# mattoverby/admm-elastic-sca

Hardware: AMD Instinct MI355X
Metric: ADMM iters/sec x #elements, 1M-tet Neo-Hookean; 1/2/4/8 MI355X (higher is better)
Workload: dtype f64

## Files before the change

admm-elastic-sca_amd/csrc/abi_setup.inc:

```

static void reset_frames(admm_hip_ctx *ctx) {
    for (int j = 0; j < ADMM_MAX_SHAPES; ++j) {
        for (int k = 0; k < 12; ++k) ctx->shapes.frame[j][k] = (k == 0 || k == 4 || k == 8) ? 1.0 : 0.0;
        ctx->shapes.framed[j] = 0;
    }
}

int admm_hip_create(admm_hip_ctx **out, int device_id) {
    if (!out) return ADMM_ERR_ARG;
    *out = nullptr;
    admm_hip_ctx *ctx = new admm_hip_ctx();
    ctx->device_id = device_id;
    if (device_id >= 0) {
        int count = 0;
        hipError_t e = hipGetDeviceCount(&count);
        if (e != hipSuccess || count <= device_id) {
            fprintf(stderr, "admm_hip: no HIP device %d (%s, %d devices) -- refusing to run without a GPU\n", device_id, hipGetErrorString(e), count);
            delete ctx;
            return ADMM_ERR_HIP;
        }
        if (hipSetDevice(device_id) != hipSuccess) { delete ctx; return ADMM_ERR_HIP; }
        if (hipStreamCreate(&ctx->stream) != hipSuccess) { delete ctx; return ADMM_ERR_HIP; }
        ctx->own_stream = true;
    }
// ... 6 lines not shown
    ctx->graph_enabled = false;
#endif
    if (const char *g = getenv("ADMM_HIP_GRAPH_COMM")) ctx->graph_comm = atoi(g) != 0;
    if (const char *g = getenv("ADMM_HIP_BWD_NW")) { const int v = atoi(g); if (v == 4 || v == 8 || v == 16) ctx->bwd_nw = v; }
    if (const char *g = getenv("ADMM_HIP_FWD_SMALL_K")) ctx->fwd_small_k = atoi(g);
    if (const char *g = getenv("ADMM_HIP_BWD_SMALL_K")) ctx->bwd_small_k = atoi(g);
    if (const char *g = getenv("ADMM_HIP_TREE_SEARCH")) ctx->tree_search = atoi(g) != 0;
    if (const char *g = getenv("ADMM_HIP_STATE_DIRECT")) ctx->state_direct_max_nodes = atoi(g);
    if (const char *g = getenv("ADMM_HIP_LOCAL_MULTI")) ctx->local_multi = atoi(g) != 0;
    if (const char *g = getenv("ADMM_HIP_TOP_BWD_ALL")) ctx->top_bwd_needed_only = atoi(g) == 0;
    if (const char *g = getenv("ADMM_HIP_ROOT_FUSE_K")) ctx->root_fuse_k = std::min(atoi(g), (int)admm_dev::ROOT_KCHUNK);
    if (const char *g = getenv("ADMM_HIP_FRAME_GRAPH")) ctx->frame_graph_on = atoi(g) != 0;
    if (const char *g = getenv("ADMM_HIP_BWD_SMALL_NW")) { const int v = atoi(g); if (v == 2 || v == 4 || v == 8 || v == 16) ctx->bwd_small_nw = v; }
    if (const char *g = getenv("ADMM_HIP_XCD")) ctx->xcd_min_supernodes = atoi(g);
    if (const char *g = getenv("ADMM_HIP_TET_ORDER")) ctx->tet_order = atoi(g) != 0;
    if (const char *g = getenv("ADMM_HIP_TET_ORDER_MIN")) ctx->tet_order_min_blocks = atoi(g);
    if (const char *g = getenv("ADMM_HIP_FUSE_ANCHORS")) ctx->fuse_anchor_tail = atoi(g) != 0;
    if (const char *g = getenv("ADMM_HIP_FACTOR")) ctx->device_factor = std::string(g) != "host";
    if (const char *g = getenv("ADMM_HIP_BWD_CW2_MIN")) ctx->bwd_cw2_min_cols = atoi(g);
    if (const char *g = getenv("ADMM_HIP_BWD_CW2_MAX")) ctx->bwd_cw2_max_cols = atoi(g);
    if (const char *g = getenv("ADMM_HIP_PRERED")) ctx->tet_prered = atoi(g) != 0;
    if (const char *g = getenv("ADMM_HIP_STATE_ZEROCOPY")) ctx->state_zero_copy = atoi(g) != 0;
    if (const char *g = getenv("ADMM_HIP_TPB")) { const int v = atoi(g); if (v == 4 || v == 8 || v == 16 || v == 32 || v == 64) ctx->tet_tpb = v; }
    if (const char *g = getenv("ADMM_HIP_KEEP_Z")) ctx->keep_z_user = atoi(g) != 0;
    if (const char *g = getenv("ADMM_HIP_BWD_NW_MIN_COLS")) ctx->bwd_nw_min_cols = atoi(g);
    if (const char *g = getenv("ADMM_HIP_FWD_NW16_TILES")) ctx->fwd_nw16_max_tiles = atoi(g);
    if (const char *g = getenv("ADMM_HIP_FWD_NW4")) ctx->fwd_nw4_kmax = atoi(g);
    if (const char *g = getenv("ADMM_HIP_FWD_NW8")) ctx->fwd_nw8_kmax = atoi(g);
    if (const char *g = getenv("ADMM_HIP_DENSE_MAX")) ctx->dense_max = atoi(g);
    if (const char *g = getenv("ADMM_HIP_ROOT_INVERSE")) ctx->root_inverse = atoi(g) != 0;
    if (const char *g = getenv("ADMM_HIP_DIST_TOP")) ctx->dist_top_wanted = atoi(g) != 0 ? 1 : 0;
    if (const char *g = getenv("ADMM_HIP_DIST_TOP_MIN_NODES")) ctx->dist_top_min_nodes = atoi(g);
    if (const char *g = getenv("ADMM_HIP_SWEEP_FUSE")) ctx->sweep_fuse = atoi(g) != 0;
    *out = ctx;
    return ADMM_OK;
}

void admm_hip_destroy(admm_hip_ctx *ctx) {
    if (!ctx) return;
    if (ctx->device_id >= 0) {
        (void)hipSetDevice(ctx->device_id);
        (void)hipDeviceSynchronize();
        free_device(ctx);
        for (hipEvent_t e : ctx->evpool) (void)hipEventDestroy(e);
        for (hipEvent_t e : ctx->evpool_prev) (void)hipEventDestroy(e);
        comm_release(ctx);
        for (double *h : {ctx->h_gen_dx, ctx->h_gen_u, ctx->h_gen_z, ctx->h_gen_q}) if (h) (void)hipHostFree(h);
        if (ctx->gen_ev) (void)hipEventDestroy(ctx->gen_ev);
        if (ctx->h_state) (void)hipHostFree(ctx->h_state);
        if (ctx->state_in_ev) (void)hipEventDestroy(ctx->state_in_ev);
        if (ctx->own_stream && ctx->stream) (void)hipStreamDestroy(ctx->stream);
    }
    delete ctx;
}

const char *admm_hip_last_error(const admm_hip_ctx *ctx) { return ctx ? ctx->err.c_str() : "null context"; }

int admm_hip_set_stream(admm_hip_ctx *ctx, void *s) {
    if (!ctx || ctx->device_id < 0) return ADMM_ERR_ARG;
    if (ctx->stream) { HIPCHK(hipSetDevice(ctx->device_id)); (void)hipStreamSynchronize(ctx->stream); }
    if (ctx->own_stream && ctx->stream) (void)hipStreamDestroy(ctx->stream);
    ctx->own_stream = false;
    ctx->stream = (hipStream_t)s;
    if (!s) { HIPCHK(hipStreamCreate(&ctx->stream)); ctx->own_stream = true; }
    return ADMM_OK;
}
// ... 664 lines not shown
```

admm-elastic-sca_amd/csrc/ctx.hpp:

```cpp
#pragma once
#include <hip/hip_runtime_api.h>

#include <algorithm>
#include <chrono>
#include <cmath>
#include <cstdarg>
#include <cstdio>
#include <cstring>
#include <numeric>
#include <string>
#include <vector>

#include "../../include/admm_hip.h"
#include "factor.hpp"
#include "dev_types.hpp"
#include "mesh_host.hpp"

namespace admm_lib {

inline double now_s() { return std::chrono::duration<double>(std::chrono::steady_clock::now().time_since_epoch()).count(); }

struct Batch {
    int kind = 0, n_total = 0, n_local = 0;
    std::vector<int32_t> local;
// ... 125 lines not shown
    int root_sn = -1, root_k = 0, root_first = 0, root_r0 = 0, root_r1 = 0; int64_t root_foff = 0;
    bool tet_order = true; int tet_order_min_blocks = 3072;
    int64_t frames = 0;
    int merge_small = 0;
    bool fuse_anchor_tail = true;
    bool device_factor = true, device_numeric = false;
    bool keep_z = true, keep_z_user = true;
    bool state_zero_copy = true;
    int tet_tpb = 0;
    bool tet_prered = true;
    int n_comm_top = 0, n_comm_slots = 0;
    int *d_comm_top = nullptr, *d_comm_slots = nullptr; unsigned char *d_comm_mine = nullptr, *d_base_mask = nullptr, *d_keep_mask = nullptr;
    double *d_comm_buf = nullptr;
    bool root_inverse = true;
    int dense_max = 2048; bool dense = false; std::vector<double> Ainv; double *d_ainv = nullptr;
    bool graph_enabled = true, graph_forced = false; hipGraph_t iter_graph = nullptr; hipGraphExec_t iter_exec = nullptr;
    bool frame_graph_on = true; hipGraph_t frame_graph = nullptr; hipGraphExec_t frame_exec = nullptr; int frame_iters = 0, last_step_iters = -1;
    bool local_multi = true;
    int state_direct_max_nodes = 12288; double *h_state = nullptr, *h_state_dev = nullptr; size_t h_state_cap = 0; int *d_iperm = nullptr; hipEvent_t state_in_ev = nullptr; bool state_in_pending = false;
    std::vector<std::pair<const char *, size_t> > pinned;
    std::vector<double> bounce;
    bool tree_search = true;
    bool top_bwd_needed_only = true;
    int root_fuse_k = 2048;
    int fwd_small_k = 64, bwd_small_k = 64;
    int bwd_cw2_min_cols = 8192, bwd_cw2_max_cols = 16384;
    int bwd_nw = 8, bwd_small_nw = 4;
    int xcd_min_supernodes = 16;
    int bwd_nw_min_cols = 4096, fwd_nw16_max_tiles = 512;
    int fwd_nw4_kmax = 200, fwd_nw8_kmax = 400;
    bool sweep_fuse = true;
    int fuse_cut = -1, n_fuse = 0, fuse_lds = 0;
    int *d_fuse_rec = nullptr; int64_t *d_fuse_off = nullptr;
    int64_t graph_launches = 0;
    bool graphs_stale = false;
    bool graph_comm = false;
    bool res_on = false, res_ready = false;
    double tol_r = 0.0, tol_s = 0.0; int check_every = 1;
    double *d_res = nullptr; int res_cap = 0, res_n = 0;
    double *d_res_slots = nullptr, *d_res_s = nullptr, *d_res_partial = nullptr; int res_partial_n = 0;
    bool en_ready = false; double *d_en_out = nullptr, *d_en_npart = nullptr; long long *d_en_cnt = nullptr;
    bool obj_on = false; int obj_cap = 0, obj_n = 0; double *d_obj = nullptr;
    bool gr_ready = false, gr_csr_ready = false; double *d_gr_cf = nullptr, *d_gr_out = nullptr;
    int *d_gr_ptr[2] = {nullptr, nullptr}, *d_gr_stride[2] = {nullptr, nullptr}; long long *d_gr_off[2] = {nullptr, nullptr};
    bool rx_ready = false; double *d_rx_el = nullptr, *d_rx_node = nullptr, *d_rx_part = nullptr; int *d_rx_blk = nullptr; long long *d_rx_count = nullptr; void *d_rx_rec = nullptr;
    int *d_rx_ptr[2] = {nullptr, nullptr}, *d_rx_stride[2] = {nullptr, nullptr}; long long *d_rx_off[2] = {nullptr, nullptr};
    int aa_m = 0, aa_cap_m = 0, aa_nblk = 0, aa_log_cap = 0, aa_log_n = 0; long long aa_T = 0; bool aa_ran = false;
    void *d_aa_seg = nullptr, *d_aa_state = nullptr; admm_hip_acceleration_record *d_aa_log = nullptr;
    double *d_aa_sin = nullptr, *d_aa_ring = nullptr, *d_aa_part = nullptr;

    admm_hip_project_fn project_hook = nullptr; void *project_user = nullptr;
    int64_t n_gen_rows = 0;
    double *d_gen_dx = nullptr, *d_gen_q = nullptr;
    double *h_gen_dx = nullptr, *h_gen_u = nullptr, *h_gen_z = nullptr, *h_gen_q = nullptr;
    std::vector<double> h_gen_u_prev, h_gen_z_prev; double *d_gen_q2 = nullptr, *d_gen_r2 = nullptr;
    hipEvent_t gen_ev = nullptr;
    bool timing = false; int timing_stride = 1; int ev_timed = 0; int timing_frame = 0;
    std::vector<hipEvent_t> evpool;
    size_t ev_used = 0; int ev_iters = 0; bool ev_pending = false;
    std::vector<hipEvent_t> evpool_prev; size_t ev_used_prev = 0; int ev_iters_prev = 0, ev_timed_prev = 0; bool ev_pending_prev = false;
    admm_hip_timing last_timing{};
};

namespace admm_lib {

int fail(admm_hip_ctx *c, int code, const char *fmt, ...);
// ... 40 lines not shown
```

admm-elastic-sca_amd/csrc/kernels_global.hpp:

```cpp
#pragma once
#include <hip/hip_runtime.h>
#include <stdint.h>
#include "dev_types.hpp"

namespace admm_dev {


__global__ void prologue_kernel(int ndof, double dt, Gravity gr, const double *__restrict__ x, double *__restrict__ v,
                                const double *__restrict__ m, double *__restrict__ mxbar, double *__restrict__ xcur) {
    const int i = blockIdx.x * blockDim.x + threadIdx.x;
    if (i >= ndof) return;
    const int c = i % 3;
    double vi = v[i];
    for (int k = 0; k < gr.n; ++k) vi += (dt * gr.g[k][c]);
    v[i] = vi;
    const double xb = x[i] + dt * vi;
    mxbar[i] = m[i] * xb;
    xcur[i] = xb;
}

__global__ void xbar_kernel(int ndof, double dt, const double *__restrict__ x, const double *__restrict__ v,
                            const double *__restrict__ m, double *__restrict__ mxbar, double *__restrict__ xcur) {
    const int i = blockIdx.x * blockDim.x + threadIdx.x;
    if (i >= ndof) return;
    const double xb = x[i] + dt * v[i];
    mxbar[i] = m[i] * xb;
    xcur[i] = xb;
}

__global__ void explicit_const_kernel(int n, const int *__restrict__ idx, double dt, double gx, double gy, double gz, double *__restrict__ v) {
    const int i = blockIdx.x * blockDim.x + threadIdx.x;
    if (i >= n) return;
    const int node = idx ? idx[i] : i;
    v[3 * (size_t)node] += (dt * gx); v[3 * (size_t)node + 1] += (dt * gy); v[3 * (size_t)node + 2] += (dt * gz);
}

// ... 587 lines not shown
                    for (int c = 0; c < CW; ++c) { acc[c][0] += pf[c] * v[0]; acc[c][1] += pf[c] * v[1]; acc[c][2] += pf[c] * v[2]; }
                    q += 64;
                }
                for (; q < rc; q += 64) {
                    const int i = r0 + q;
                    double p[CW];
#pragma unroll
                    for (int c = 0; c < CW; ++c) p[c] = (j0 + c < k && i >= j0 + c) ? Pj[i + (size_t)f * c] : 0.0;
                    const double *v = &vs[3 * q];
#pragma unroll
                    for (int c = 0; c < CW; ++c) { acc[c][0] += p[c] * v[0]; acc[c][1] += p[c] * v[1]; acc[c][2] += p[c] * v[2]; }
                }
                for (; q < rc; q += 64) {
                    const int i = r0 + q;
                    const double *v = &vs[3 * q];
#pragma unroll
                    for (int c = 0; c < CW; ++c) { const double p = (j0 + c < k && i >= j0 + c) ? Pj[i + (size_t)f * c] : 0.0; acc[c][0] += p * v[0]; acc[c][1] += p * v[1]; acc[c][2] += p * v[2]; }
                }
            }
        }
    }
    double v[3 * CW];
#pragma unroll
    for (int c = 0; c < CW; ++c) { v[3 * c] = acc[c][0]; v[3 * c + 1] = acc[c][1]; v[3 * c + 2] = acc[c][2]; }
    int base = 0, cnt = 3 * CW;
    wave_sum_transpose<3 * CW, 32>(v, lane, base, cnt);
    if (cnt >= 1) {
        const int c = base / 3, m = base - 3 * c;
        if (j0 + c < k) X[3 * (size_t)(first + j0 + c) + m] = v[0];
    }
    ADMM_SWEEP_STAMP(2);
}

template <bool CG2>
__global__ __launch_bounds__(256) void root_gather_kernel(int k, int first, int64_t foff, FactorDev F, const double *__restrict__ y, const double *__restrict__ C, double *__restrict__ T, double *__restrict__ Xzero = nullptr) {
    const int j = blockIdx.x * 256 + threadIdx.x;
    if (j >= k) return;
    if (Xzero) { Xzero[3 * (size_t)j] = 0.0; Xzero[3 * (size_t)j + 1] = 0.0; Xzero[3 * (size_t)j + 2] = 0.0; }
    double s0, s1, s2;
    child_sum<CG2>(F, foff + j, C, s0, s1, s2);
    const double *src = y + 3 * (size_t)(first + j);
    double *t = T + 3 * (size_t)j;
    t[0] = src[0] - s0; t[1] = src[1] - s1; t[2] = src[2] - s2;
}

__global__ __launch_bounds__(256) void dense_solve_kernel(int n, const double *__restrict__ Ainv, const double *__restrict__ b, double *__restrict__ X) {
    const int wave = threadIdx.x >> 6, lane = threadIdx.x & 63;
    const int i = blockIdx.x * 4 + wave;
    if (i >= n) return;
    const double *row = Ainv + (size_t)i * n;
    double v[3] = {0.0, 0.0, 0.0};
    int j = lane;
    for (; j + 448 < n; j += 512) {
        double a[8];
#pragma unroll
        for (int q = 0; q < 8; ++q) a[q] = row[j + 64 * q];
#pragma unroll
        for (int q = 0; q < 8; ++q) { const double *bj = b + 3 * (size_t)(j + 64 * q); v[0] += a[q] * bj[0]; v[1] += a[q] * bj[1]; v[2] += a[q] * bj[2]; }
    }
    for (; j + 192 < n; j += 256) {
        double a[4];
#pragma unroll
        for (int q = 0; q < 4; ++q) a[q] = row[j + 64 * q];
#pragma unroll
        for (int q = 0; q < 4; ++q) { const double *bj = b + 3 * (size_t)(j + 64 * q); v[0] += a[q] * bj[0]; v[1] += a[q] * bj[1]; v[2] += a[q] * bj[2]; }
    }
// ... 61 lines not shown
```

admm-elastic-sca_amd/csrc/launch.inc:

```

int max_lbfgs_iters(const Batch &b) { return b.max_iter; }

#ifdef ADMM_TET_PROFILE
float *g_trace_base; int g_trace_cap, g_trace_n, g_trace_count;
void tet_trace_next(hipStream_t st) {
    float *p = (g_trace_base && g_trace_count < g_trace_cap) ? g_trace_base + 2 * (size_t)g_trace_count * g_trace_n : nullptr;
    ++g_trace_count;
    hipMemcpyToSymbolAsync(HIP_SYMBOL(admm_dev::g_tet_trace), &p, sizeof(p), 0, hipMemcpyHostToDevice, st);
}
#endif
bool friction_on(const admm_hip_ctx *ctx) {
    for (int q = 0; q < ctx->shapes.n; ++q) if (ctx->shapes.mu[q] > 0.0) return true;
    return false;
}

bool moving_friction_on(const admm_hip_ctx *ctx) {
    for (int q = 0; q < ctx->shapes.n; ++q) {
        const int id = ctx->shapes.type[q] == ADMM_SHAPE_MESH ? (int)ctx->shapes.par[q][3] : -1;
        const admm_hip_ctx::MeshMove *mv = id >= 0 && id < (int)ctx->mesh_move.size() ? &ctx->mesh_move[id] : nullptr;
        if (mv && !ctx->mesh_role[id].body_nodes.empty() && mv->body_mu > 0.0) return true;
        if (!(ctx->shapes.mu[q] > 0.0)) continue;
        if (mv && mv->has_vel) return true;
        for (int k = 0; k < 9; ++k) if (ctx->shapes.motion[q][k] != 0.0) return true;
    }
// ... 340 lines not shown
                    return NWB != 2 || CW == 4;
                }); });
            }
        };
        if (ctx->n_fuse)
            hipLaunchKernelGGL(solve_fwd_subtree_kernel, dim3(ctx->n_fuse), dim3(64 * SUB_WAVES), ctx->fuse_lds, ctx->stream, (const int *)ctx->d_fuse_rec,
                               (const int64_t *)ctx->d_fuse_off, (const double *)ctx->d_panels, (const double *)ctx->d_y, ctx->d_w, ctx->d_c);
        forward(ctx->levels, ctx->stream);
        if (!ctx->levels_top.empty()) {
            const int n = ctx->n_comm_top + ctx->n_comm_slots;
            if (ex0) HIPCHK(hipEventRecord(ex0, ctx->stream));
            if (n > 0) {
                hipLaunchKernelGGL(shard_pack_kernel, dim3((n + 255) / 256), dim3(256), 0, ctx->stream, ctx->n_comm_top, (const int *)ctx->d_comm_top, ctx->n_comm_slots,
                                   (const int *)ctx->d_comm_slots, (const unsigned char *)ctx->d_comm_mine, (const double *)ctx->d_y, (const double *)ctx->d_c, ctx->d_comm_buf);
                TRY(do_allreduce(ctx, ctx->d_comm_buf, 3 * (int64_t)n));
                hipLaunchKernelGGL(shard_unpack_kernel, dim3((n + 255) / 256), dim3(256), 0, ctx->stream, ctx->n_comm_top, (const int *)ctx->d_comm_top, ctx->n_comm_slots,
                                   (const int *)ctx->d_comm_slots, (const double *)ctx->d_comm_buf, ctx->d_y, ctx->d_c);
            }
            if (ex1) HIPCHK(hipEventRecord(ex1, ctx->stream));
            if (ctx->dist_top) {
                const int k = ctx->root_k, nr = ctx->root_r1 - ctx->root_r0;
                double *T = ctx->d_w + 3 * (size_t)ctx->root_first, *Xr = ctx->d_xcur + 3 * (size_t)ctx->root_first;
                hipLaunchKernelGGL((root_gather_kernel<CG2>), dim3((k + 255) / 256), dim3(256), 0, ctx->stream, k, ctx->root_first, ctx->root_foff, F, (const double *)ctx->d_y, (const double *)ctx->d_c, T, Xr);
                if (nr > 0) hipLaunchKernelGGL((root_product_kernel<false, false>), dim3((nr + ROOT_ROWS - 1) / ROOT_ROWS), dim3(64 * ROOT_ROWS), 0, ctx->stream, k, nr, root_inv_ld(k),
                                               (const double *)(ctx->d_panels + ctx->dev_root_inv_off[ctx->root_sn]), (const double *)T, Xr + 3 * (size_t)ctx->root_r0, 0, (int64_t)0, F, (const double *)nullptr);
                if (ex2) HIPCHK(hipEventRecord(ex2, ctx->stream));
                TRY(do_allreduce(ctx, Xr, 3 * (int64_t)k));
                if (ex3) HIPCHK(hipEventRecord(ex3, ctx->stream));
            } else forward(ctx->levels_top, ctx->stream);
        }
        if (mid) HIPCHK(hipEventRecord(mid, ctx->stream));
        if (!ctx->levels_top.empty() && !ctx->dist_top) backward(ctx->levels_top, ctx->stream);
        backward(ctx->levels, ctx->stream);
        HIPCHK(hipGetLastError());
        if (bad_pair) return fail(ctx, ADMM_ERR_STATE, "backward sweep: no kernel for a level's (columns per wave, waves per block) pair");
        return ADMM_OK;
    };
    return F.cg4 ? sweeps(std::true_type{}) : sweeps(std::false_type{});
}

int shard_sync_x(admm_hip_ctx *ctx) {
    if (ctx->levels_top.empty()) return ADMM_OK;
    const int n3 = 3 * ctx->n_nodes;
    hipLaunchKernelGGL(admm_dev::shard_mask_nodes_kernel, dim3((n3 + 255) / 256), dim3(256), 0, ctx->stream, ctx->n_nodes, (const unsigned char *)ctx->d_keep_mask, ctx->d_xcur);
    TRY(do_allreduce(ctx, ctx->d_xcur, (int64_t)n3));
    HIPCHK(hipGetLastError());
    return ADMM_OK;
}


int ensure_residual_buffers(admm_hip_ctx *ctx, int iters) {
    if (ctx->res_ready && iters <= ctx->res_cap) return ADMM_OK;
    HIPCHK(hipSetDevice(ctx->device_id));
    if (!ctx->res_ready) {
        int64_t slots = 0; int maxn = 0;
        for (Batch &b : ctx->batches) {
            if (b.kind == ADMM_KIND_GENERIC) {
                std::vector<double> coef(b.g_sval.size());
                for (size_t i = 0; i < coef.size(); ++i) { const double w = b.g_roww[b.g_srow_b[i]]; coef[i] = b.g_sval[i] * (w * w); }
                TRY(upload(ctx, &b.d_g_scoef_res, coef));
                slots += b.g_lslots;
                continue;
            }
            const int rows = ADMM_KIND_ROWS[b.kind], nl = std::max(b.n_local, 1);
            b.res_fused = ((b.kind >= ADMM_KIND_TET_LINEAR && b.kind <= ADMM_KIND_TET_STVK) || b.kind == ADMM_KIND_ANCHOR) && (b.prered || getenv("ADMM_HIP_RES_UNFUSED") == nullptr);
            if (b.res_fused) {
// ... 113 lines not shown
```

admm-elastic-sca_amd/csrc/upload.inc:

```

template <class T> std::vector<T> permute_nodes(const std::vector<T> &h, const std::vector<int> &perm, int comps) {
    std::vector<T> o(h.size());
    for (size_t i = 0; i < perm.size(); ++i) for (int c = 0; c < comps; ++c) o[comps * i + c] = h[comps * (size_t)perm[i] + c];
    return o;
}

#ifdef ADMM_SWEEP_PROFILE
unsigned long long *g_swp_base; size_t g_swp_wgs; std::vector<int> g_swp_meta;
#endif
int fuse_subtrees(admm_hip_ctx *ctx, const std::vector<int> *own, int want, std::vector<char> &fused) {
    using namespace admm_dev;
    const Factor &F = ctx->F;
    const int ns = (int)F.sn.size();
    fused.assign(ns, 0);
    ctx->fuse_cut = -1; ctx->n_fuse = 0; ctx->fuse_lds = 0;
    const bool verbose = getenv("ADMM_HIP_VERBOSE") != nullptr;
    const char *why_off = !ctx->sweep_fuse ? "ADMM_HIP_SWEEP_FUSE=0" : (F.cg4.empty() ? "front rows with more than four contributions" : (F.levels.empty() ? "no cut level" : nullptr));
    if (why_off) { if (verbose) fprintf(stderr, "admm_hip: plan fused off (%s)\n", why_off); return ADMM_OK; }
    auto mine = [&](int s) { return !own || (*own)[s] == want; };
    hipDeviceProp_t prop;
    HIPCHK(hipGetDeviceProperties(&prop, ctx->device_id));
    const int cus = std::max(prop.multiProcessorCount, 1);
    const int lds_cap = (int)std::min<size_t>(prop.sharedMemPerBlock, prop.maxSharedMemoryPerMultiProcessor / 2);
    const int kcap = std::min(std::min(ctx->fwd_small_k, ctx->bwd_small_k), FWD_SMALL_KMAX);
    int cut = -1;
    for (int l = 0; l < (int)F.levels.size(); ++l) {
        bool narrow = true;
        for (int s : F.levels[l]) if (mine(s) && F.sn[s].ncols > kcap) narrow = false;
        if (!narrow) break;
        int roots = 0;
        for (int s = 0; s < ns; ++s) {
            const int p = F.sn[s].parent;
            if (mine(s) && F.sn[s].level <= l && p >= 0 && F.sn[p].level > l) ++roots;
        }
        if (roots >= 2 * cus) cut = l;
    }
    if (cut < 0) { if (verbose) fprintf(stderr, "admm_hip: plan fused off (no cut level)\n"); return ADMM_OK; }
    std::vector<std::vector<int> > children(ns);
    for (int s = 0; s < ns; ++s) if (F.sn[s].parent >= 0) children[F.sn[s].parent].push_back(s);
    std::vector<int> local_slot(F.n_slots, -1);
    struct Rec { std::vector<int> v; double bytes; std::vector<int> members; };
    std::vector<Rec> recs;
    int lds_max = 0, left = 0;
    int lv_min = 0, lv_max = 0, maxin = 0, skip = 0, empty = 0;
    for (int t = 0; t < ns; ++t) {
        const int p = F.sn[t].parent;
        if (!mine(t) || F.sn[t].level > cut || p < 0 || F.sn[p].level <= cut) continue;
        std::vector<int> mem, stack{t};
        while (!stack.empty()) { const int s = stack.back(); stack.pop_back(); mem.push_back(s); for (int c : children[s]) stack.push_back(c); }
        const int nlv = F.sn[t].level + 1;
        std::vector<std::vector<int> > bylv(nlv);
        for (int s : mem) bylv[F.sn[s].level].push_back(s);
        for (auto &v : bylv) std::sort(v.begin(), v.end());
        bool ok = true;
        for (int s : mem) if (!mine(s) || F.sn[s].root_inv_off >= 0) ok = false;
        int cdoubles = 0;
        for (int s : mem) if (s != t) { for (int q = 0; q < F.sn[s].nrows; ++q) local_slot[F.sn[s].slot_off + q] = cdoubles + 3 * q; cdoubles += 3 * F.sn[s].nrows; }
        std::vector<int> lvp{0}, items, maps;
        int n_items = 0;
        for (int l = 0; l < nlv; ++l) {
            if (bylv[l].empty()) continue;
            for (int s : bylv[l]) {
                const Supernode &S = F.sn[s];
                const int f = S.ncols + S.nrows;
                int moff = -1;
                if (!children[s].empty()) {
                    moff = (int)maps.size();
                    for (int fr = 0; fr < f; ++fr) for (int e = 0; e < 4; ++e) {
                        const int g = F.cg4[4 * (size_t)(S.front_off + fr) + e];
                        const int o = g < 0 ? -1 : local_slot[g];
                        if (g >= 0 && o < 0) ok = false;
                        maps.push_back(o);
                    }
                }
                const int cdst = s == t ? -1 : (S.nrows ? local_slot[S.slot_off] : 0);
                int it[SUB_ITEM] = {};
                it[SUB_K] = S.ncols; it[SUB_R] = S.nrows; it[SUB_FIRST] = S.first; it[SUB_MAP] = moff; it[SUB_CDST] = cdst;
                sub_split64(ctx->dev_panel_off[s], it + SUB_POFF);
                for (int tile = 0; tile < (f + 63) / 64; ++tile) {
                    it[SUB_TILE] = tile;
                    items.insert(items.end(), it, it + SUB_ITEM);
                    ++n_items;
                }
            }
            lvp.push_back(n_items);
        }
        for (int s : mem) if (s != t) for (int q = 0; q < F.sn[s].nrows; ++q) local_slot[F.sn[s].slot_off + q] = -1;
        if (!ok) { ++left; continue; }
        const int nl = (int)lvp.size() - 1;
        const int item0 = (SUB_HDR + nl + 1 + 3) & ~3, map0 = item0 + SUB_ITEM * n_items;
        const int n_ints = (map0 + (int)maps.size() + 3) & ~3;
        std::vector<int> v(n_ints, 0);
        const int64_t rs = F.sn[t].slot_off;
        const int cbuf = n_ints / 2;
        const int ts_off = cbuf + cdoubles;
        v[SUB_LEVELS] = nl; v[SUB_ITEM0] = item0; v[SUB_CBUF] = cbuf; v[SUB_TS] = ts_off; sub_split64(rs, &v[SUB_ROOT_SLOT]);
        for (int l = 0; l <= nl; ++l) v[SUB_HDR + l] = lvp[l];
        for (size_t q = 0; q < items.size(); ++q) {
            v[item0 + q] = items[q];
            if (q % SUB_ITEM == SUB_MAP && items[q] >= 0) v[item0 + q] += map0;
        }
        std::copy(maps.begin(), maps.end(), v.begin() + map0);
        const int lds = 8 * (ts_off + 3 * 64 * SUB_WAVES);
        if (lds > lds_cap) { ++left; continue; }
        double bytes = 0.0;
        for (int s : mem) { const double k = F.sn[s].ncols, f = k + F.sn[s].nrows; bytes += 8.0 * (f * k - 0.5 * k * (k - 1)); }
        lds_max = std::max(lds_max, lds);
        if (verbose) {
            lv_min = recs.empty() ? nl : std::min(lv_min, nl); lv_max = std::max(lv_max, nl);
            for (size_t q = 0; q < maps.size(); q += 4) maxin = std::max(maxin, (maps[q] >= 0) + (maps[q + 1] >= 0) + (maps[q + 2] >= 0) + (maps[q + 3] >= 0));
            for (int s : mem) if (s != t) { skip += F.sn[F.sn[s].parent].level - F.sn[s].level >= 2; empty += F.sn[s].nrows == 0; }
        }
        recs.push_back({std::move(v), bytes, std::move(mem)});
    }
    if (verbose)
        fprintf(stderr, "admm_hip: plan fused cut %d subtrees %d left %d lds %d cap %d levels %d..%d maxin %d skip %d empty %d\n", cut, (int)recs.size(), left, lds_max, lds_cap,
                lv_min, lv_max, maxin, skip, empty);
    if (recs.empty()) return ADMM_OK;
    std::stable_sort(recs.begin(), recs.end(), [](const Rec &a, const Rec &b) { return a.bytes > b.bytes; });
    std::vector<int> all; std::vector<int64_t> off{0};
    for (const Rec &r : recs) { all.insert(all.end(), r.v.begin(), r.v.end()); off.push_back((int64_t)all.size()); for (int s : r.members) fused[s] = 1; }
    TRY(upload(ctx, &ctx->d_fuse_rec, all)); TRY(upload(ctx, &ctx->d_fuse_off, off));
    ctx->fuse_cut = cut; ctx->n_fuse = (int)recs.size(); ctx->fuse_lds = lds_max;
    return ADMM_OK;
}

int upload_factor(admm_hip_ctx *ctx) {
#ifdef ADMM_SWEEP_PROFILE
    g_swp_wgs = 0; g_swp_meta.clear();
#endif
    Factor &F = ctx->F;
    const int ns = (int)F.sn.size();
    std::vector<int> first(ns), ncols(ns), nrows(ns);
    std::vector<int64_t> poff(ns), roff(ns), soff(ns), foff(ns);
    for (int s = 0; s < ns; ++s) { first[s] = F.sn[s].first; ncols[s] = F.sn[s].ncols; nrows[s] = F.sn[s].nrows; poff[s] = ctx->dev_panel_off[s]; roff[s] = F.sn[s].rows_off; soff[s] = F.sn[s].slot_off; foff[s] = F.sn[s].front_off; }
    TRY(dalloc(ctx, &ctx->d_panels, (size_t)std::max<int64_t>(ctx->dev_panels_size, 1)));
    TRY(panels_to_device(ctx));
    TRY(upload(ctx, &ctx->d_sn_first, first)); TRY(upload(ctx, &ctx->d_sn_ncols, ncols)); TRY(upload(ctx, &ctx->d_sn_nrows, nrows));
    TRY(upload(ctx, &ctx->d_sn_panel_off, poff)); TRY(upload(ctx, &ctx->d_sn_rows_off, roff)); TRY(upload(ctx, &ctx->d_sn_slot_off, soff));
    TRY(upload(ctx, &ctx->d_rows, F.rows));
    TRY(upload(ctx, &ctx->d_sn_front_off, foff));
    TRY(upload(ctx, &ctx->d_cg_ptr, F.cg_ptr)); TRY(upload(ctx, &ctx->d_cg_slot, F.cg_slot));
    ctx->d_cg4 = nullptr;
    if (!F.cg4.empty()) TRY(upload(ctx, &ctx->d_cg4, F.cg4));
    TRY(dalloc(ctx, &ctx->d_c, 3 * (size_t)std::max<int64_t>(F.n_slots, 1)));
    ctx->d_ainv = nullptr;
    if (ctx->dense) TRY(upload(ctx, &ctx->d_ainv, ctx->Ainv));
    ctx->levels.assign(F.levels.size(), LevelDev());
    std::vector<int> level_kmax(F.levels.size(), 0);
    for (size_t l = 0; l < F.levels.size(); ++l) for (int s : F.levels[l]) level_kmax[l] = std::max(level_kmax[l], F.sn[s].ncols);
    const int fwd_small_k = std::min(ctx->fwd_small_k, admm_dev::FWD_SMALL_KMAX);
    const bool subtree = ctx->shard_mode == 1 && ctx->world > 1;
    ctx->levels_top.assign(subtree ? F.levels.size() : 0, LevelDev());
    struct Pass { int want; std::vector<LevelDev> *into; };
    std::vector<Pass> passes;
    if (subtree) { passes.push_back({ctx->rank, &ctx->levels}); passes.push_back({-1, &ctx->levels_top}); }
    else passes.push_back({0, &ctx->levels});
    const std::vector<int> *own = subtree ? &ctx->sn_owner : nullptr;
    std::vector<char> fused;
    TRY(fuse_subtrees(ctx, own, subtree ? ctx->rank : 0, fused));
    std::vector<char> top_needed;
    std::vector<int> top_provider;
    if (subtree) {
        std::vector<std::vector<char> > need;
        top_needs(ctx, need, top_provider);
        top_needed = need[ctx->rank];
        if (getenv("ADMM_HIP_VERBOSE")) {
            int nt = 0, nn = 0;
            for (int s2 = 0; s2 < ns; ++s2) if (ctx->sn_owner[s2] < 0) { ++nt; nn += top_needed[s2] ? 1 : 0; }
            fprintf(stderr, "admm_hip: rank %d: backward sweep over %d of the %d top supernodes\n", ctx->rank, nn, nt);
        }
    }
    for (const Pass &ps : passes) {
        for (size_t l = 0; l < F.levels.size(); ++l) {
            LevelDev &L = (*ps.into)[l];
            std::vector<admm_dev::SweepItem> sm, bg, bw;
            L.level = (int)l; L.mbytes = 0.0;
            const bool fwd_small = level_kmax[l] <= fwd_small_k, bwd_small = level_kmax[l] <= ctx->bwd_small_k;
            L.bwd_cw = bwd_small ? 4 : BWD_BIG_CW;
            int level_cols = 0;
            for (int s : F.levels[l]) if (!own || (*own)[s] == ps.want) level_cols += F.sn[s].ncols;
            L.bwd_nw = bwd_small ? ctx->bwd_small_nw : (level_cols >= ctx->bwd_nw_min_cols ? ctx->bwd_nw : 4);
            if (!bwd_small && ctx->bwd_cw2_min_cols > 0 && level_cols > ctx->bwd_cw2_min_cols && level_cols <= ctx->bwd_cw2_max_cols) L.bwd_cw = 2;
            for (int s : F.levels[l]) {
                if (own && (*own)[s] != ps.want) continue;
                const Supernode &S = F.sn[s];
                admm_dev::SweepItem it{};
                it.s = s; it.k = S.ncols; it.r = S.nrows; it.first = S.first;
                it.panel_off = ctx->dev_panel_off[s]; it.front_off = S.front_off; it.slot_off = S.slot_off; it.rows_off = S.rows_off;
                const int f = S.ncols + S.nrows;
                const int tiles = (f + 63) / 64;
                L.mbytes += 8e-6 * ((double)f * S.ncols - 0.5 * (double)S.ncols * (S.ncols - 1));
                if (S.root_inv_off >= 0 && ctx->root_inverse) {
                    L.roots.push_back({S.ncols, S.first, S.front_off, ctx->dev_root_inv_off[s]});
                    continue;
                }
                const bool in_fused = ps.want >= 0 && fused[s];
                if (!in_fused) for (int t = 0; t < tiles; ++t) { it.part = t; if (fwd_small) sm.push_back(it); else bg.push_back(it); }
                const int chunks = (S.ncols + L.bwd_nw * L.bwd_cw - 1) / (L.bwd_nw * L.bwd_cw);
                if (subtree && ps.want < 0 && !top_needed[s]) continue;
                for (int c = 0; c < chunks; ++c) { it.part = c; bw.push_back(it); }
            }
            if (ctx->xcd_min_supernodes > 0) { xcd_order(sm, admm_dev::FWD_SMALL_WAVES, ctx->xcd_min_supernodes); xcd_order(bg, 1, ctx->xcd_min_supernodes); xcd_order(bw, 1, ctx->xcd_min_supernodes); }
            L.n_small = (int)sm.size(); L.n_big = (int)bg.size(); L.n_bwd = (int)bw.size();
            int kmax = 0;
            for (const admm_dev::SweepItem &q : bg) kmax = std::max(kmax, q.k);
            L.big_nw = (int)bg.size() <= ctx->fwd_nw16_max_tiles ? 16 : (kmax <= ctx->fwd_nw4_kmax ? 4 : (kmax <= ctx->fwd_nw8_kmax ? 8 : 16));
            if (getenv("ADMM_HIP_VERBOSE")) {
                using namespace admm_dev;
                const char *pass = ps.want < 0 ? "top" : "own";
                const int kchunk = L.big_nw == 16 ? FwdBig<16>::KCHUNK : (L.big_nw == 8 ? FwdBig<8>::KCHUNK : FwdBig<4>::KCHUNK);
                int fmax = 0;
                for (const SweepItem &q : bw) fmax = std::max(fmax, q.k + q.r);
                fprintf(stderr, "admm_hip: plan %s level %zu: fwd wave %d block %d big_nw %d kmax %d chunks %d | bwd cw %d nw %d items %d fmax %d rchunks %d | cg4 %d\n",
                        pass, l, L.n_small, L.n_big, L.big_nw, kmax, (kmax + kchunk - 1) / kchunk, L.bwd_cw, L.bwd_nw, L.n_bwd, fmax, (fmax + BWD_RCHUNK - 1) / BWD_RCHUNK,
                        F.cg4.empty() ? 0 : 1);
                for (const LevelDev::Root &R : L.roots)
                    fprintf(stderr, "admm_hip: plan %s level %zu: root k %d %s chunks %d\n", pass, l, R.k, R.k <= ctx->root_fuse_k ? "fused" : "gather",
                            (R.k + ROOT_KCHUNK - 1) / ROOT_KCHUNK);
            }
#ifdef ADMM_SWEEP_PROFILE
            {
                const int list = ps.want < 0 ? 100 : (&ps - &passes[0]);
                auto reg = [&](std::vector<admm_dev::SweepItem> &v, int group, int tag) {
                    if (v.empty()) return;
                    const int n_wg = ((int)v.size() + group - 1) / group;
                    for (size_t i = 0; i < v.size(); ++i) v[i].pad2 = (v[i].k || v[i].r) ? (long long)(g_swp_wgs + i / group) : -1;
                    for (int q : {tag, (int)l, n_wg, (int)(L.mbytes * 1024), list, (int)g_swp_wgs}) g_swp_meta.push_back(q);
                    g_swp_wgs += n_wg;
                };
                reg(sm, admm_dev::FWD_SMALL_WAVES, 0); reg(bg, 1, L.big_nw); reg(bw, 1, 100 + 10 * L.bwd_cw + (L.bwd_nw == 16 ? 6 : L.bwd_nw));
            }
#endif
// ... 421 lines not shown
```

Measured before the change: 1.440 billion.

## Fuse backward triangular solve over small subtrees into one LDS-resident kernel

Adds a backward-sweep counterpart to the existing fused forward subtree solve. For each subtree below the cut level that fits in LDS, it builds a per-block record of levels, members, tasks and staging. A single kernel then walks the subtree's levels top-down, keeping the solved x values in LDS and using block barriers instead of per-level launches. Those supernodes are dropped from the per-level backward kernels, which cuts launch and global-memory round-trips for the many small bottom levels. The cost is a host-side record build and validation, plus LDS pressure and barrier-serialised levels inside each block.

After: 1.458 billion (median of 6 runs). +1.2%, better.

```diff
diff --git a/admm-elastic-sca_amd/csrc/abi_setup.inc b/admm-elastic-sca_amd/csrc/abi_setup.inc
--- a/admm-elastic-sca_amd/csrc/abi_setup.inc
+++ b/admm-elastic-sca_amd/csrc/abi_setup.inc
@@ -62,6 +62,7 @@
     if (const char *g = getenv("ADMM_HIP_DIST_TOP")) ctx->dist_top_wanted = atoi(g) != 0 ? 1 : 0;
     if (const char *g = getenv("ADMM_HIP_DIST_TOP_MIN_NODES")) ctx->dist_top_min_nodes = atoi(g);
     if (const char *g = getenv("ADMM_HIP_SWEEP_FUSE")) ctx->sweep_fuse = atoi(g) != 0;
+    if (const char *g = getenv("ADMM_HIP_SWEEP_FUSE_BWD")) ctx->sweep_fuse_bwd = atoi(g) != 0;
     *out = ctx;
     return ADMM_OK;
 }
diff --git a/admm-elastic-sca_amd/csrc/bwd_record.hpp b/admm-elastic-sca_amd/csrc/bwd_record.hpp
--- /dev/null
+++ b/admm-elastic-sca_amd/csrc/bwd_record.hpp
@@ -0,0 +1,91 @@
+#pragma once
+#include <stdint.h>
+#include <stdio.h>
+#include <vector>
+
+namespace admm_dev {
+
+constexpr int BS_LEVELS = 0, BS_NMEM = 1, BS_MEM0 = 2, BS_NTASK = 3, BS_TASK0 = 4, BS_XBUF = 5, BS_VBUF = 6, BS_END = 7, BS_NSTAGE = 8, BS_STAGE0 = 9, BS_HDR = 12;
+constexpr int BS_K = 0, BS_R = 1, BS_FIRST = 2, BS_XOFF = 3, BS_VOFF = 4, BS_ROW0 = 5, BS_POFF = 6 , BS_MEM = BS_POFF + 2;
+constexpr int64_t BS_MAX_NODES = (int64_t)1 << 29;
+constexpr int BS_KMAX = 64;
+
+inline bool bwd_record_check(const int *rec, int64_t n_ints, int64_t n_nodes, int64_t panels_size, char *msg, int msg_len) {
+    auto bad = [&](const char *what, long long a, long long b) { snprintf(msg, (size_t)msg_len, "backward subtree record: %s (%lld, %lld)", what, a, b); return false; };
+    if (n_ints < BS_HDR || (n_ints & 3)) return bad("record size", n_ints, 0);
+    const int64_t nl = rec[BS_LEVELS], nm = rec[BS_NMEM], m0 = rec[BS_MEM0], nt = rec[BS_NTASK], t0 = rec[BS_TASK0];
+    const int64_t xb = rec[BS_XBUF], vb = rec[BS_VBUF], end = rec[BS_END], nst = rec[BS_NSTAGE], s0 = rec[BS_STAGE0];
+    if (n_nodes > BS_MAX_NODES) return bad("too many nodes", n_nodes, 0);
+    if (nl < 1 || nm < 1 || nt < 1 || nst < 1) return bad("empty", nl, nm);
+    if (BS_HDR + 3 * (nl + 1) > m0 || m0 + BS_MEM * nm > t0 || t0 + nt > s0 || s0 + nst > n_ints) return bad("areas of the record overlap", m0, t0);
+    if (2 * xb < n_ints || xb > vb || vb > end) return bad("LDS areas out of order", xb, vb);
+    const int64_t xsize = vb - xb, vsize = end - vb;
+    const int *lvm = rec + BS_HDR, *lvt = rec + BS_HDR + nl + 1, *lvs = rec + BS_HDR + 2 * (nl + 1);
+    if (lvm[0] != 0 || lvm[nl] != nm || lvt[0] != 0 || lvt[nl] != nt || lvs[0] != 0 || lvs[nl] != nst) return bad("level pointers", lvm[nl], lvt[nl]);
+    for (int64_t l = 0; l < nl; ++l) if (lvm[l] >= lvm[l + 1] || lvt[l] >= lvt[l + 1] || lvs[l] >= lvs[l + 1]) return bad("empty level", l, lvm[l]);
+    for (int64_t l = 0; l < nl; ++l) if (3 * ((int64_t)lvs[l + 1] - lvs[l]) > vsize) return bad("staged level beyond the staging area", l, lvs[l + 1] - lvs[l]);
+    std::vector<int> level_of(nm, -1);
+    for (int64_t l = 0; l < nl; ++l) for (int q = lvm[l]; q < lvm[l + 1]; ++q) level_of[q] = (int)l;
+    std::vector<int> x_owner((size_t)(xsize / 3 + 1), -1);
+    for (int64_t q = 0; q < nm; ++q) {
+        const int *M = rec + m0 + BS_MEM * q;
+        const int64_t k = M[BS_K], r = M[BS_R], first = M[BS_FIRST], xo = M[BS_XOFF], vo = M[BS_VOFF], r0 = M[BS_ROW0];
+        const int64_t poff = (int64_t)(((uint64_t)(uint32_t)M[BS_POFF + 1] << 32) | (uint32_t)M[BS_POFF]);
+        if (k < 1 || k > BS_KMAX || r < 0) return bad("member shape", q, k);
+        if (first < 0 || first + k > n_nodes) return bad("member columns outside the system", q, first);
+        if (poff < 0 || poff + (k + r) * k > panels_size) return bad("panel offset", q, poff);
+        if (vo < 0 || vo % 3 || vo + 3 * (k + r) > vsize) return bad("staging offset", q, vo);
+        if (r0 < lvs[level_of[q]] || r0 + k + r > lvs[level_of[q] + 1]) return bad("stage rows outside the member's level", q, r0);
+        if (vo != 3 * (r0 - lvs[level_of[q]])) return bad("staging offset is not the stage rows'", q, vo);
+        if (xo < -1 || (xo >= 0 && (xo % 3 || xo + 3 * k > xsize))) return bad("x offset", q, xo);
+        if (xo >= 0) for (int64_t j = 0; j < k; ++j) {
+            if (x_owner[xo / 3 + j] >= 0) return bad("x slot written twice", q, x_owner[xo / 3 + j]);
+            x_owner[xo / 3 + j] = (int)q;
+        }
+    }
+    for (int64_t l = 0; l < nl; ++l) {
+        int64_t rows = 0;
+        for (int q = lvm[l]; q < lvm[l + 1]; ++q) rows += (int64_t)rec[m0 + BS_MEM * q + BS_K] + rec[m0 + BS_MEM * q + BS_R];
+        if (rows != (int64_t)lvs[l + 1] - lvs[l]) return bad("stage rows of a level are not its members' rows", l, rows);
+    }
+    for (int64_t l = 0; l < nl; ++l)
+        for (int a = lvm[l]; a < lvm[l + 1]; ++a) for (int b = a + 1; b < lvm[l + 1]; ++b) {
+            const int *A = rec + m0 + BS_MEM * a, *B = rec + m0 + BS_MEM * b;
+            const int64_t a0 = A[BS_VOFF], a1 = a0 + 3 * ((int64_t)A[BS_K] + A[BS_R]), b0 = B[BS_VOFF], b1 = b0 + 3 * ((int64_t)B[BS_K] + B[BS_R]);
+            if (a0 < b1 && b0 < a1) return bad("staged vectors overlap", a, b);
+        }
+    std::vector<int> seen((size_t)nm * 16, 0);
+    for (int64_t l = 0; l < nl; ++l) for (int t = lvt[l]; t < lvt[l + 1]; ++t) {
+        const int v = rec[t0 + t], q = v >> 4, g = v & 15;
+        if (v < 0 || q >= nm) return bad("task member", t, q);
+        if (level_of[q] != l) return bad("task outside its member's level", t, q);
+        if (4 * g >= rec[m0 + BS_MEM * q + BS_K]) return bad("task beyond the member's columns", t, g);
+        if (seen[(size_t)q * 16 + g]++) return bad("column written twice", q, 4 * g);
+    }
+    for (int64_t q = 0; q < nm; ++q) for (int g = 0; 4 * g < rec[m0 + BS_MEM * q + BS_K]; ++g)
+        if (!seen[(size_t)q * 16 + g]) return bad("column never written", q, 4 * g);
+    for (int64_t q = 0; q < nm; ++q) {
+        const int *M = rec + m0 + BS_MEM * q;
+        const int *st = rec + s0 + M[BS_ROW0];
+        for (int i = 0; i < M[BS_K] + M[BS_R]; ++i) {
+            const int64_t e = st[i];
+            if (i < M[BS_K]) {
+                if (e != -1 - (2 * ((int64_t)M[BS_FIRST] + i) + 1)) return bad("own column not staged from w", q, i);
+            } else if (e >= 0) {
+                if (e % 3 || e + 3 > xsize || x_owner[e / 3] < 0) return bad("row outside the x area", q, e);
+                if (level_of[x_owner[e / 3]] >= level_of[q]) return bad("row of a member that is not at a higher level", q, x_owner[e / 3]);
+            } else {
+                const int64_t n = -1 - e, node = n >> 1;
+                if (n & 1) return bad("front row staged from w", q, i);
+                if (node >= n_nodes) return bad("row outside the system", q, node);
+                for (int64_t p = 0; p < nm; ++p) {
+                    const int *P = rec + m0 + BS_MEM * p;
+                    if (node >= P[BS_FIRST] && node < (int64_t)P[BS_FIRST] + P[BS_K]) return bad("row read from global x lies inside the subtree", q, node);
+                }
+            }
+        }
+    }
+    return true;
+}
+
+}
diff --git a/admm-elastic-sca_amd/csrc/ctx.hpp b/admm-elastic-sca_amd/csrc/ctx.hpp
--- a/admm-elastic-sca_amd/csrc/ctx.hpp
+++ b/admm-elastic-sca_amd/csrc/ctx.hpp
@@ -181,6 +181,9 @@
     bool sweep_fuse = true;
     int fuse_cut = -1, n_fuse = 0, fuse_lds = 0;
     int *d_fuse_rec = nullptr; int64_t *d_fuse_off = nullptr;
+    bool sweep_fuse_bwd = true;
+    int n_fuse_bwd = 0, fuse_bwd_lds = 0;
+    int *d_fuse_bwd_rec = nullptr; int64_t *d_fuse_bwd_off = nullptr;
     int64_t graph_launches = 0;
     bool graphs_stale = false;
     bool graph_comm = false;
diff --git a/admm-elastic-sca_amd/csrc/kernels_global.hpp b/admm-elastic-sca_amd/csrc/kernels_global.hpp
--- a/admm-elastic-sca_amd/csrc/kernels_global.hpp
+++ b/admm-elastic-sca_amd/csrc/kernels_global.hpp
@@ -2,6 +2,7 @@
 #include <hip/hip_runtime.h>
 #include <stdint.h>
 #include "dev_types.hpp"
+#include "bwd_record.hpp"
 
 namespace admm_dev {
 
@@ -655,6 +656,115 @@
     ADMM_SWEEP_STAMP(2);
 }
 
+__device__ __forceinline__ bool bwd_sub_counts(int f, int k, int j0, int i, int c) { return j0 + c < k && i < f && i >= j0 + c; }
+__device__ __forceinline__ void bwd_sub_request(const double *Pj, int f, int k, int j0, int i, long long (&p)[4]) {
+#pragma unroll
+    for (int c = 0; c < 4; ++c) {
+        const unsigned off = bwd_sub_counts(f, k, j0, i, c) ? (unsigned)(i + f * c) << 3 : 0u;
+        p[c] = __double_as_longlong(*reinterpret_cast<const double *>(reinterpret_cast<const char *>(Pj) + off));
+    }
+}
+__global__ __launch_bounds__(64 * SUB_WAVES, 6) void solve_bwd_kernel_subtree(const int *__restrict__ recs, const int64_t *__restrict__ rec_off, const double *__restrict__ panels,
+                                                                           const double *__restrict__ W, double *X, int bmask) {
+    extern __shared__ double sub_lds[];
+    int *meta = reinterpret_cast<int *>(sub_lds);
+    const int wave = sub_uniform(threadIdx.x >> 6), lane = threadIdx.x & 63;
+    {
+        const int64_t o0 = rec_off[blockIdx.x], o1 = rec_off[blockIdx.x + 1];
+        const int4 *src = reinterpret_cast<const int4 *>(recs + o0);
+        int4 *dst = reinterpret_cast<int4 *>(meta);
+        const int n4 = (int)((o1 - o0) >> 2);
+        for (int q = threadIdx.x; q < n4; q += 64 * SUB_WAVES) dst[q] = src[q];
+    }
+    __syncthreads();
+    const int n_lv = meta[BS_LEVELS], mem0 = meta[BS_MEM0], task0 = meta[BS_TASK0];
+    double *xs = sub_lds + meta[BS_XBUF];
+    double *vs = sub_lds + meta[BS_VBUF];
+    const int *lvt = meta + BS_HDR + n_lv + 1, *lvs = meta + BS_HDR + 2 * (n_lv + 1);
+    const int *stage = meta + meta[BS_STAGE0];
+    auto staged = [&](int e, double (&a)[3]) {
+        const bool lds = e >= 0;
+        const int n = -1 - e;
+        const bool w = (n & 1) != 0;
+        const double *gp = (w ? W : (const double *)X) + 3 * (size_t)(lds ? 0 : n >> 1);
+        const double *lp = xs + (lds ? e : 0);
+        const double g0 = gp[0], g1 = gp[1], g2 = gp[2], l0 = lp[0], l1 = lp[1], l2 = lp[2];
+        a[0] = lds ? -l0 : (w ? g0 : -g0); a[1] = lds ? -l1 : (w ? g1 : -g1); a[2] = lds ? -l2 : (w ? g2 : -g2);
+    };
+    struct Task { int k, f, first, j0, jc0, xoff, voff; const double *Pj; };
+    auto task = [&](int t) {
+        const int tv = sub_uniform(meta[task0 + t]);
+        const int *M = meta + mem0 + BS_MEM * (tv >> 4);
+        Task g;
+        g.k = sub_uniform(M[BS_K]); g.f = g.k + sub_uniform(M[BS_R]); g.first = sub_uniform(M[BS_FIRST]);
+        g.xoff = sub_uniform(M[BS_XOFF]); g.voff = sub_uniform(M[BS_VOFF]);
+        g.j0 = 4 * (tv & 15); g.jc0 = g.j0 & ~bmask;
+        g.Pj = panels + sub_join64(sub_uniform(M[BS_POFF]), sub_uniform(M[BS_POFF + 1])) + (size_t)g.f * g.j0;
+        return g;
+    };
+    for (int lv = 0; lv < n_lv; ++lv) {
+        const int te = lvt[lv + 1];
+        int t = lvt[lv] + wave, ib = 0;
+        Task g{};
+        long long A[4], B[4];
+        if (t < te) { g = task(t); ib = g.jc0; bwd_sub_request(g.Pj, g.f, g.k, g.j0, ib + lane, A); }
+        {
+            const int *st = stage + lvs[lv];
+            const int ns = lvs[lv + 1] - lvs[lv];
+            constexpr int NT = 64 * SUB_WAVES;
+            for (int q = threadIdx.x; q < ns; q += 2 * NT) {
+                const bool two = q + NT < ns;
+                const int q1 = two ? q + NT : q;
+                const int e0 = st[q], e1 = st[q1];
+                double a[3], b[3];
+                staged(e0, a); staged(e1, b);
+                vs[3 * q] = a[0]; vs[3 * q + 1] = a[1]; vs[3 * q + 2] = a[2];
+                if (two) { vs[3 * q1] = b[0]; vs[3 * q1 + 1] = b[1]; vs[3 * q1 + 2] = b[2]; }
+            }
+        }
+        asm volatile("s_waitcnt lgkmcnt(0)\n\ts_barrier" ::: "memory");
+        double acc[4][3];
+#pragma unroll
+        for (int c = 0; c < 4; ++c) { acc[c][0] = 0.0; acc[c][1] = 0.0; acc[c][2] = 0.0; }
+        auto step = [&](long long (&cur)[4], long long (&nxt)[4]) {
+            int tn = t, in = ib + 64;
+            Task gn = g;
+            if (in >= g.f) { tn = t + SUB_WAVES; if (tn < te) { gn = task(tn); in = gn.jc0; } }
+            bwd_sub_request(gn.Pj, gn.f, gn.k, gn.j0, in + lane, nxt);
+            const int i = ib + lane;
+            if (i < g.f) {
+                const double *vi = vs + g.voff + 3 * i;
+#pragma unroll
+                for (int c = 0; c < 4; ++c) {
+                    const double p = __longlong_as_double(cur[c] & (bwd_sub_counts(g.f, g.k, g.j0, i, c) ? -1ll : 0ll));
+                    acc[c][0] += p * vi[0]; acc[c][1] += p * vi[1]; acc[c][2] += p * vi[2];
+                }
+            }
+            if (tn != t) {
+                double s[12];
+#pragma unroll
+                for (int c = 0; c < 4; ++c) { s[3 * c] = acc[c][0]; s[3 * c + 1] = acc[c][1]; s[3 * c + 2] = acc[c][2]; acc[c][0] = 0.0; acc[c][1] = 0.0; acc[c][2] = 0.0; }
+                int base = 0, cnt = 12;
+                wave_sum_transpose<12, 32>(s, lane, base, cnt);
+                if (cnt >= 1) {
+                    const int c = base / 3, m = base - 3 * c;
+                    if (g.j0 + c < g.k) {
+                        X[3 * (size_t)(g.first + g.j0 + c) + m] = s[0];
+                        if (g.xoff >= 0) xs[g.xoff + 3 * (g.j0 + c) + m] = s[0];
+                    }
+                }
+            }
+            t = tn; ib = in; g = gn;
+        };
+        while (t < te) {
+            step(A, B);
+            if (t >= te) break;
+            step(B, A);
+        }
+        asm volatile("s_waitcnt lgkmcnt(0)\n\ts_barrier" ::: "memory");
+    }
+}
+
 template <bool CG2>
 __global__ __launch_bounds__(256) void root_gather_kernel(int k, int first, int64_t foff, FactorDev F, const double *__restrict__ y, const double *__restrict__ C, double *__restrict__ T, double *__restrict__ Xzero = nullptr) {
     const int j = blockIdx.x * 256 + threadIdx.x;
diff --git a/admm-elastic-sca_amd/csrc/launch.inc b/admm-elastic-sca_amd/csrc/launch.inc
--- a/admm-elastic-sca_amd/csrc/launch.inc
+++ b/admm-elastic-sca_amd/csrc/launch.inc
@@ -396,6 +396,9 @@
         if (mid) HIPCHK(hipEventRecord(mid, ctx->stream));
         if (!ctx->levels_top.empty() && !ctx->dist_top) backward(ctx->levels_top, ctx->stream);
         backward(ctx->levels, ctx->stream);
+        if (ctx->n_fuse_bwd)
+            hipLaunchKernelGGL(solve_bwd_kernel_subtree, dim3(ctx->n_fuse_bwd), dim3(64 * SUB_WAVES), ctx->fuse_bwd_lds, ctx->stream, (const int *)ctx->d_fuse_bwd_rec,
+                               (const int64_t *)ctx->d_fuse_bwd_off, (const double *)ctx->d_panels, (const double *)ctx->d_w, ctx->d_xcur, 4 * ctx->bwd_small_nw - 1);
         HIPCHK(hipGetLastError());
         if (bad_pair) return fail(ctx, ADMM_ERR_STATE, "backward sweep: no kernel for a level's (columns per wave, waves per block) pair");
         return ADMM_OK;
diff --git a/admm-elastic-sca_amd/csrc/upload.inc b/admm-elastic-sca_amd/csrc/upload.inc
--- a/admm-elastic-sca_amd/csrc/upload.inc
+++ b/admm-elastic-sca_amd/csrc/upload.inc
@@ -8,15 +8,62 @@
 #ifdef ADMM_SWEEP_PROFILE
 unsigned long long *g_swp_base; size_t g_swp_wgs; std::vector<int> g_swp_meta;
 #endif
-int fuse_subtrees(admm_hip_ctx *ctx, const std::vector<int> *own, int want, std::vector<char> &fused) {
+int bwd_subtree_record(const admm_hip_ctx *ctx, const std::vector<std::vector<int> > &bylv, const std::vector<std::vector<int> > &children, std::vector<int> &node_x,
+                       std::vector<int> &v) {
+    using namespace admm_dev;
+    const Factor &F = ctx->F;
+    std::vector<int> lvm{0}, lvt{0}, lvs{0}, mem, tasks, stage;
+    int xd = 0, vmax = 0, nm = 0;
+    for (int l = (int)bylv.size() - 1; l >= 0; --l) {
+        if (bylv[l].empty()) continue;
+        int vd = 0;
+        for (int s : bylv[l]) {
+            const Supernode &S = F.sn[s];
+            int it[BS_MEM] = {};
+            it[BS_K] = S.ncols; it[BS_R] = S.nrows; it[BS_FIRST] = S.first; it[BS_XOFF] = -1; it[BS_VOFF] = vd; it[BS_ROW0] = (int)stage.size();
+            sub_split64(ctx->dev_panel_off[s], it + BS_POFF);
+            vd += 3 * (S.ncols + S.nrows);
+            for (int j = 0; j < S.ncols; ++j) stage.push_back(-1 - (2 * (S.first + j) + 1));
+            for (int q = 0; q < S.nrows; ++q) { const int node = F.rows[S.rows_off + q]; stage.push_back(node_x[node] >= 0 ? node_x[node] : -1 - 2 * node); }
+            if (!children[s].empty()) {
+                it[BS_XOFF] = xd;
+                for (int j = 0; j < S.ncols; ++j) node_x[S.first + j] = xd + 3 * j;
+                xd += 3 * S.ncols;
+            }
+            for (int g = 0; 4 * g < S.ncols; ++g) tasks.push_back(nm * 16 + g);
+            mem.insert(mem.end(), it, it + BS_MEM);
+            ++nm;
+        }
+        vmax = std::max(vmax, vd);
+        lvm.push_back(nm); lvt.push_back((int)tasks.size()); lvs.push_back((int)stage.size());
+    }
+    for (const std::vector<int> &lv : bylv) for (int s : lv) if (!children[s].empty()) for (int j = 0; j < F.sn[s].ncols; ++j) node_x[F.sn[s].first + j] = -1;
+    const int nl = (int)lvm.size() - 1;
+    const int mem0 = (BS_HDR + 3 * (nl + 1) + 3) & ~3, task0 = mem0 + BS_MEM * nm, stage0 = task0 + (int)tasks.size();
+    const int n_ints = (stage0 + (int)stage.size() + 3) & ~3;
+    v.assign(n_ints, 0);
+    const int xbuf = n_ints / 2, vbuf = xbuf + xd, end = vbuf + vmax;
+    v[BS_LEVELS] = nl; v[BS_NMEM] = nm; v[BS_MEM0] = mem0; v[BS_NTASK] = (int)tasks.size(); v[BS_TASK0] = task0; v[BS_XBUF] = xbuf; v[BS_VBUF] = vbuf; v[BS_END] = end;
+    v[BS_NSTAGE] = (int)stage.size(); v[BS_STAGE0] = stage0;
+    for (int l = 0; l <= nl; ++l) { v[BS_HDR + l] = lvm[l]; v[BS_HDR + nl + 1 + l] = lvt[l]; v[BS_HDR + 2 * (nl + 1) + l] = lvs[l]; }
+    std::copy(mem.begin(), mem.end(), v.begin() + mem0);
+    std::copy(tasks.begin(), tasks.end(), v.begin() + task0);
+    std::copy(stage.begin(), stage.end(), v.begin() + stage0);
+    return 8 * end;
+}
+
+int fuse_subtrees(admm_hip_ctx *ctx, const std::vector<int> *own, int want, std::vector<char> &fused, std::vector<char> &fused_bwd) {
     using namespace admm_dev;
     const Factor &F = ctx->F;
     const int ns = (int)F.sn.size();
-    fused.assign(ns, 0);
+    fused.assign(ns, 0); fused_bwd.assign(ns, 0);
     ctx->fuse_cut = -1; ctx->n_fuse = 0; ctx->fuse_lds = 0;
+    ctx->n_fuse_bwd = 0; ctx->fuse_bwd_lds = 0;
     const bool verbose = getenv("ADMM_HIP_VERBOSE") != nullptr;
+    const char *why_bwd_off = !ctx->sweep_fuse ? "ADMM_HIP_SWEEP_FUSE=0" : (!ctx->sweep_fuse_bwd ? "ADMM_HIP_SWEEP_FUSE_BWD=0" : (F.n > BS_MAX_NODES ? "too many nodes" : nullptr));
+    auto bwd_off = [&](const char *why) { if (verbose) fprintf(stderr, "admm_hip: plan fused_bwd off (%s)\n", why); };
     const char *why_off = !ctx->sweep_fuse ? "ADMM_HIP_SWEEP_FUSE=0" : (F.cg4.empty() ? "front rows with more than four contributions" : (F.levels.empty() ? "no cut level" : nullptr));
-    if (why_off) { if (verbose) fprintf(stderr, "admm_hip: plan fused off (%s)\n", why_off); return ADMM_OK; }
+    if (why_off) { if (verbose) fprintf(stderr, "admm_hip: plan fused off (%s)\n", why_off); bwd_off(why_bwd_off ? why_bwd_off : "no fused forward subtrees"); return ADMM_OK; }
     auto mine = [&](int s) { return !own || (*own)[s] == want; };
     hipDeviceProp_t prop;
     HIPCHK(hipGetDeviceProperties(&prop, ctx->device_id));
@@ -35,17 +82,20 @@
         }
         if (roots >= 2 * cus) cut = l;
     }
-    if (cut < 0) { if (verbose) fprintf(stderr, "admm_hip: plan fused off (no cut level)\n"); return ADMM_OK; }
+    if (cut < 0) { if (verbose) fprintf(stderr, "admm_hip: plan fused off (no cut level)\n"); bwd_off(why_bwd_off ? why_bwd_off : "no fused forward subtrees"); return ADMM_OK; }
     std::vector<std::vector<int> > children(ns);
     for (int s = 0; s < ns; ++s) if (F.sn[s].parent >= 0) children[F.sn[s].parent].push_back(s);
     std::vector<int> local_slot(F.n_slots, -1);
-    struct Rec { std::vector<int> v; double bytes; std::vector<int> members; };
+    struct Rec { std::vector<int> v; double bytes; std::vector<int> members; std::vector<int> bwd; };
     std::vector<Rec> recs;
     int lds_max = 0, left = 0;
+    std::vector<int> node_x(F.n, -1);
+    int bwd_lds_max = 0, n_bwd = 0, candidates = 0;
     int lv_min = 0, lv_max = 0, maxin = 0, skip = 0, empty = 0;
     for (int t = 0; t < ns; ++t) {
         const int p = F.sn[t].parent;
         if (!mine(t) || F.sn[t].level > cut || p < 0 || F.sn[p].level <= cut) continue;
+        ++candidates;
         std::vector<int> mem, stack{t};
         while (!stack.empty()) { const int s = stack.back(); stack.pop_back(); mem.push_back(s); for (int c : children[s]) stack.push_back(c); }
         const int nlv = F.sn[t].level + 1;
@@ -111,17 +161,36 @@
             for (size_t q = 0; q < maps.size(); q += 4) maxin = std::max(maxin, (maps[q] >= 0) + (maps[q + 1] >= 0) + (maps[q + 2] >= 0) + (maps[q + 3] >= 0));
             for (int s : mem) if (s != t) { skip += F.sn[F.sn[s].parent].level - F.sn[s].level >= 2; empty += F.sn[s].nrows == 0; }
         }
-        recs.push_back({std::move(v), bytes, std::move(mem)});
+        std::vector<int> bwd;
+        if (!why_bwd_off) {
+            const int bl = bwd_subtree_record(ctx, bylv, children, node_x, bwd);
+            if (bl > lds_cap) bwd.clear();
+            else {
+                char msg[256];
+                if (!bwd_record_check(bwd.data(), (int64_t)bwd.size(), F.n, ctx->dev_panels_size, msg, (int)sizeof msg)) return fail(ctx, ADMM_ERR_STATE, "%s", msg);
+                bwd_lds_max = std::max(bwd_lds_max, bl); ++n_bwd;
+            }
+        }
+        recs.push_back({std::move(v), bytes, std::move(mem), std::move(bwd)});
     }
     if (verbose)
         fprintf(stderr, "admm_hip: plan fused cut %d subtrees %d left %d lds %d cap %d levels %d..%d maxin %d skip %d empty %d\n", cut, (int)recs.size(), left, lds_max, lds_cap,
                 lv_min, lv_max, maxin, skip, empty);
+    if (why_bwd_off) bwd_off(why_bwd_off);
+    else if (!n_bwd) bwd_off(recs.empty() ? "no fused forward subtrees" : "every subtree over the LDS cap");
+    else if (verbose) fprintf(stderr, "admm_hip: plan fused_bwd cut %d subtrees %d left %d lds %d cap %d\n", cut, n_bwd, candidates - n_bwd, bwd_lds_max, lds_cap);
     if (recs.empty()) return ADMM_OK;
     std::stable_sort(recs.begin(), recs.end(), [](const Rec &a, const Rec &b) { return a.bytes > b.bytes; });
     std::vector<int> all; std::vector<int64_t> off{0};
     for (const Rec &r : recs) { all.insert(all.end(), r.v.begin(), r.v.end()); off.push_back((int64_t)all.size()); for (int s : r.members) fused[s] = 1; }
     TRY(upload(ctx, &ctx->d_fuse_rec, all)); TRY(upload(ctx, &ctx->d_fuse_off, off));
     ctx->fuse_cut = cut; ctx->n_fuse = (int)recs.size(); ctx->fuse_lds = lds_max;
+    if (n_bwd) {
+        std::vector<int> ball; std::vector<int64_t> boff{0};
+        for (const Rec &r : recs) if (!r.bwd.empty()) { ball.insert(ball.end(), r.bwd.begin(), r.bwd.end()); boff.push_back((int64_t)ball.size()); for (int s : r.members) fused_bwd[s] = 1; }
+        TRY(upload(ctx, &ctx->d_fuse_bwd_rec, ball)); TRY(upload(ctx, &ctx->d_fuse_bwd_off, boff));
+        ctx->n_fuse_bwd = n_bwd; ctx->fuse_bwd_lds = bwd_lds_max;
+    }
     return ADMM_OK;
 }
 
@@ -157,8 +226,8 @@
     if (subtree) { passes.push_back({ctx->rank, &ctx->levels}); passes.push_back({-1, &ctx->levels_top}); }
     else passes.push_back({0, &ctx->levels});
     const std::vector<int> *own = subtree ? &ctx->sn_owner : nullptr;
-    std::vector<char> fused;
-    TRY(fuse_subtrees(ctx, own, subtree ? ctx->rank : 0, fused));
+    std::vector<char> fused, fused_bwd;
+    TRY(fuse_subtrees(ctx, own, subtree ? ctx->rank : 0, fused, fused_bwd));
     std::vector<char> top_needed;
     std::vector<int> top_provider;
     if (subtree) {
@@ -199,6 +268,7 @@
                 if (!in_fused) for (int t = 0; t < tiles; ++t) { it.part = t; if (fwd_small) sm.push_back(it); else bg.push_back(it); }
                 const int chunks = (S.ncols + L.bwd_nw * L.bwd_cw - 1) / (L.bwd_nw * L.bwd_cw);
                 if (subtree && ps.want < 0 && !top_needed[s]) continue;
+                if (ps.want >= 0 && fused_bwd[s]) continue;
                 for (int c = 0; c < chunks; ++c) { it.part = c; bw.push_back(it); }
             }
             if (ctx->xcd_min_supernodes > 0) { xcd_order(sm, admm_dev::FWD_SMALL_WAVES, ctx->xcd_min_supernodes); xcd_order(bg, 1, ctx->xcd_min_supernodes); xcd_order(bw, 1, ctx->xcd_min_supernodes); }
```
